# scroll-tech/scroll-prover

Hardware: AMD Instinct MI355X
Metric: BN254 MSM G1-adds/sec at k=26 (higher is better)
Workload: dtype u32 (9x29-bit limbs of 254-bit Montgomery integers; v_mad_u64_u32); 1 GPU; BN254 G1 Pippenger MSM, 2^26 uniform random scalars x synthetic SRS points, inputs resident in HBM; point-range shards over 1 GPU(s), RCCL all-gather of 96-B partials; log_n=26, window_bits=22, windows=12, parallelism=point-range x1, one rank per GPU, srs_window_tables=True

## Files before the change

include/mi355zk.h:

```cpp
#ifndef MI355ZK_H
#define MI355ZK_H
#include <stdint.h>
#ifdef __cplusplus
extern "C" {
#endif

#define MI355_OK 0
#define MI355_EBADARG 1
#define MI355_ENODEVICE 2
#define MI355_EOOM 3
#define MI355_EHIP 4
#define MI355_ERCCL 5

int mi355_init(int device_id);
int mi355_init_multi(const int *device_ids, int n_devices);
int mi355_device_count(int *n_out);
int mi355_shutdown(void);
const char *mi355_last_error(void);
const char *mi355_version(void);
int mi355_set_stream(void *hip_stream);
int mi355_reset_stream(void);
int mi355_synchronize(void);

int mi355_buf_alloc(uint64_t bytes, int device_slot, void **dev_ptr_out);
// ... 63 lines not shown
int mi355_fr_vec_mul_periodic_dev(void *data_dev, uint64_t n, const void *table_host, uint32_t period);
int mi355_fr_gate_eval_dev(void *dst_dev, const void *const *polys_dev, uint32_t n_polys, const void *coeffs_fr_host, const uint32_t *term_len,
                           uint32_t n_terms, const uint32_t *factor_poly, const int32_t *factor_rot, uint64_t n, int accumulate);
int mi355_fr_interleave_dev(void *dst_dev, const void *const *parts_dev, uint32_t q_parts, uint64_t n);
int mi355_fr_batch_invert_dev(void *data_dev, uint64_t n);
int mi355_fr_kate_division_dev(void *dst_dev, const void *poly_dev, uint64_t n, const void *z);
int mi355_fr_prefix_product_dev(void *dst_dev, const void *src_dev, uint64_t n, void *total_out_host);
int mi355_fr_prefix_sum_dev(void *dst_dev, const void *src_dev, uint64_t n, void *total_out_host);
int mi355_fr_lookup_multiplicities_dev(void *m_dev, uint64_t n, const void *table_dev, uint64_t table_rows, const void *const *inputs_dev,
                                       uint32_t n_inputs, uint64_t input_rows, uint32_t flags, uint64_t *missing_out);

int mi355_eval_polynomial_dev(const void *poly_dev, uint64_t n, const void *point, void *out_fr_host);
int mi355_eval_polynomial_batch_dev(const void *const *polys_dev, uint32_t batch, uint64_t n, const void *points, void *out_fr_host);
int mi355_eval_polynomial_host(const void *poly_host, uint64_t n, const void *point, void *out_fr_host);

int mi355_srs_setup_dev(void *g_dev, void *g_lagrange_dev, uint32_t k, const void *tau, const void *omega);
int mi355_g1_fixed_base_mul_dev(void *points_affine_dev, const void *scalars_dev, uint64_t n);

int mi355_g2_mul_host(const void *p_g2affine_host, const void *scalar_fr, void *out_g2affine_host);
int mi355_msm_g2_adhoc_host(const void *bases_g2affine_host, const void *scalars_host, uint64_t n, void *out_g2affine_host);
int mi355_msm_g2_dev(const void *bases_g2affine_dev, const void *scalars_dev, uint64_t n, void *out_g2affine_host);
int mi355_msm_g2_batch_dev(const void *bases_g2affine_dev, const void *const *scalars_dev, uint32_t batch, uint64_t n, void *out_g2affine_host);

int mi355_g1_fft_dev(void *points_jac_dev, uint32_t log_n, const void *omega);
int mi355_g1_fft_host(void *points_jac_host, uint32_t log_n, const void *omega);
int mi355_g_to_lagrange_dev(const void *g_affine_dev, void *g_lagrange_affine_dev, uint32_t log_n, const void *omega_inv, const void *n_inv);
int mi355_srs_downsize(uint64_t g_handle, uint32_t k, const void *omega_inv, const void *n_inv, uint64_t *g_lagrange_handle_out);
int mi355_srs_read_host(uint64_t handle, uint64_t offset, uint64_t n, void *out_affine_host);

int mi355_profile_enable(int on);
int mi355_profile_get(const char *name, double *ms_out, uint64_t *launches_out);
int mi355_profile_reset(void);
int mi355_msm_last_plan(int *c_out, int *windows_out, uint64_t *entries_out);
int mi355_msm_last_run(int *devices_out, const char **exchange_out, int *shared_tables_out, int *host_slices_out);

int mi355_debug_ws_read(const char *role, uint64_t offset, void *dst_host, uint64_t bytes);

#ifdef __cplusplus
}
#endif
#endif
```

scroll-prover_amd/_capi.py:

```python
from __future__ import annotations

import ctypes as C
import os

HERE = os.path.dirname(os.path.abspath(__file__))
LIB_PATH = os.environ.get("MI355ZK_LIB") or os.path.join(HERE, "libmi355zk.so")

OK, EBADARG, ENODEVICE, EOOM, EHIP, ERCCL = 0, 1, 2, 3, 4, 5
_vp, _u64, _u32, _int = C.c_void_p, C.c_uint64, C.c_uint32, C.c_int

SIGNATURES = {
    "mi355_init": (_int, [_int]),
    "mi355_init_multi": (_int, [C.POINTER(_int), _int]),
    "mi355_device_count": (_int, [C.POINTER(_int)]),
    "mi355_shutdown": (_int, []),
    "mi355_last_error": (C.c_char_p, []),
    "mi355_version": (C.c_char_p, []),
    "mi355_set_stream": (_int, [_vp]),
    "mi355_reset_stream": (_int, []),
    "mi355_synchronize": (_int, []),
    "mi355_buf_alloc": (_int, [_u64, _int, C.POINTER(_vp)]),
    "mi355_buf_free": (_int, [_vp]),
    "mi355_buf_trim": (_int, []),
    "mi355_buf_slot": (_int, [_vp, C.POINTER(_int)]),
# ... 45 lines not shown
    "mi355_ntt_fr_batch_host": (_int, [C.POINTER(_vp), _u32, _u32, _vp, _vp]),
    "mi355_ntt_fr_batch_dev": (_int, [C.POINTER(_vp), _u32, _u32, _vp, _vp]),
    "mi355_coset_ntt_fr_batch_dev": (_int, [C.POINTER(_vp), C.POINTER(_vp), _u32, _u32, _vp, _vp]),
    "mi355_fr_gate_eval_dev": (_int, [_vp, C.POINTER(_vp), _u32, _vp, C.POINTER(_u32), _u32, C.POINTER(_u32), C.POINTER(C.c_int32), _u64, _int]),
    "mi355_fr_interleave_dev": (_int, [_vp, C.POINTER(_vp), _u32, _u64]),
    "mi355_fr_vec_axpy_dev": (_int, [_vp, _vp, _vp, _vp, _u64]),
    "mi355_fr_vec_op_dev": (_int, [_int, _vp, _vp, _vp, _u64]),
    "mi355_fr_vec_mul_periodic_dev": (_int, [_vp, _u64, _vp, _u32]),
    "mi355_g1_fft_dev": (_int, [_vp, _u32, _vp]),
    "mi355_g1_fft_host": (_int, [_vp, _u32, _vp]),
    "mi355_g_to_lagrange_dev": (_int, [_vp, _vp, _u32, _vp, _vp]),
    "mi355_srs_load_params_file": (_int, [C.c_char_p, _u32, C.POINTER(_u32), C.POINTER(_u64), C.POINTER(_u64), _vp, _vp]),
    "mi355_srs_downsize": (_int, [_u64, _u32, _vp, _vp, C.POINTER(_u64)]),
    "mi355_srs_read_host": (_int, [_u64, _u64, _u64, _vp]),
    "mi355_fr_kate_division_dev": (_int, [_vp, _vp, _u64, _vp]),
    "mi355_fr_batch_invert_dev": (_int, [_vp, _u64]),
    "mi355_fr_prefix_product_dev": (_int, [_vp, _vp, _u64, _vp]),
    "mi355_fr_prefix_sum_dev": (_int, [_vp, _vp, _u64, _vp]),
    "mi355_fr_lookup_multiplicities_dev": (_int, [_vp, _u64, _vp, _u64, C.POINTER(_vp), _u32, _u64, _u32, C.POINTER(_u64)]),
    "mi355_eval_polynomial_dev": (_int, [_vp, _u64, _vp, _vp]),
    "mi355_eval_polynomial_batch_dev": (_int, [C.POINTER(_vp), _u32, _u64, _vp, _vp]),
    "mi355_eval_polynomial_host": (_int, [_vp, _u64, _vp, _vp]),
    "mi355_srs_setup_dev": (_int, [_vp, _vp, _u32, _vp, _vp]),
    "mi355_g1_fixed_base_mul_dev": (_int, [_vp, _vp, _u64]),
    "mi355_g2_mul_host": (_int, [_vp, _vp, _vp]),
    "mi355_msm_g2_adhoc_host": (_int, [_vp, _vp, _u64, _vp]),
    "mi355_msm_g2_dev": (_int, [_vp, _vp, _u64, _vp]),
    "mi355_msm_g2_batch_dev": (_int, [_vp, C.POINTER(_vp), _u32, _u64, _vp]),
    "mi355_profile_enable": (_int, [_int]),
    "mi355_profile_get": (_int, [C.c_char_p, C.POINTER(C.c_double), C.POINTER(_u64)]),
    "mi355_profile_reset": (_int, []),
    "mi355_debug_ws_read": (_int, [C.c_char_p, _u64, _vp, _u64]),
    "mi355_msm_last_plan": (_int, [C.POINTER(_int), C.POINTER(_int), C.POINTER(_u64)]),
    "mi355_msm_last_run": (_int, [C.POINTER(_int), C.POINTER(C.c_char_p), C.POINTER(_int), C.POINTER(_int)]),
}


class Mi355Error(RuntimeError):
    def __init__(self, code: int, msg: str):
        super().__init__(f"mi355zk error {code}: {msg}")
        self.code = code


_lib = None


def lib() -> C.CDLL:
    global _lib
    if _lib is None:
        if not os.path.exists(LIB_PATH):
            raise Mi355Error(ENODEVICE, f"{LIB_PATH} is missing: run __graft_entry__.build() (hipcc --offload-arch=gfx950); there is no CPU fallback")
        try:
            import torch
        except Exception:
            pass
        _lib = C.CDLL(LIB_PATH)
        for name, (res, args) in SIGNATURES.items():
            fn = getattr(_lib, name)
            fn.restype, fn.argtypes = res, args
    return _lib


def check(rc: int) -> None:
    if rc != OK:
        raise Mi355Error(rc, lib().mi355_last_error().decode())

# ... 38 lines not shown
```

scroll-prover_amd/csrc/lib_common.hpp:

```cpp
#pragma once
#include <hip/hip_runtime.h>
#include <stdio.h>
#include <stdlib.h>
#include <string.h>
#include <algorithm>
#include <atomic>
#include <chrono>
#include <map>
#include <memory>
#include <mutex>
#include <string>
#include <thread>
#include <condition_variable>
#include <unordered_map>
#include <vector>

#include "../../include/mi355zk.h"
#include "fp.hpp"
#include "g1.hpp"
#include "g1_29.hpp"
#include "ntt_types.hpp"

namespace mi355 {
using namespace zk;
// ... 34 lines not shown

struct Span { std::string name; hipEvent_t a, b; };
struct Ctx {
  bool inited = false;
  int slot = 0;
  std::vector<Span> spans;
  void *comm = nullptr;
  hipEvent_t ev_xchg = nullptr;
  hipEvent_t ev_xchg2 = nullptr;
  hipStream_t copy_stream = nullptr; hipEvent_t ev_copy[4] = {nullptr, nullptr, nullptr, nullptr};
  hipEvent_t ev_up_fork = nullptr;
  hipEvent_t ev_up[8] = {nullptr, nullptr, nullptr, nullptr, nullptr, nullptr, nullptr, nullptr}; uint32_t up_next = 0;
  uint32_t host_slice_min_log = 22;
  uint32_t host_batch_overlap = 1;
  uint32_t host_chunks = 8;
  int device = -1;
  hipDeviceProp_t prop;
  hipStream_t own_stream = nullptr, stream = nullptr;
  hipStream_t aux_stream[2] = {nullptr, nullptr};
  hipEvent_t ev_fork = nullptr;
  MsmSlot msm_slot[2];
  std::vector<const fe_t *> polys_stage;
  uint32_t msm_chunks = 1;
  uint32_t msm_chunk_min_log = 23;
  int last_chunks = 1;
  std::map<std::string, Buf> ws;
  std::map<std::string, NttPlan> ntt_plans;
  g1_affine_t *fixed_base_table = nullptr;
  uint32_t sort_t2 = 0;
  uint32_t seg_factor = 16;
  uint32_t sort_fb = 11;
  uint32_t sort_split = 1;
  uint32_t reduce_chains = 131072;
  uint32_t seg_fill = 40, seg_fill_segfix = 40;
  uint32_t seg_min = 16;
  uint32_t fixup_mode = 2;
  uint32_t fixup_huge_min = 2048;
  uint32_t fixup_serial_max = 32;
  uint32_t fixup_lanes_max_log = 17;
  uint32_t tail_coop_mask = 15;
  uint32_t tail_coop_max = 65536;
  uint32_t reduce_min_chunk = 4;
  uint32_t sort_t1 = 16384;
  uint32_t ntt_direct2_max_log = 25;
  uint32_t ntt_coset_fold_max_log = 26;
  uint32_t ntt_direct2_min_log = 0;
  uint32_t ntt_fold_scale = 1;
  uint32_t ntt_batch_max_log = 22;
  uint32_t ntt_two_level_max_log = 18;
  uint32_t ntt_tile_log = 11;
  bool profiling = false;
  bool trace = false;
  std::map<std::string, Prof> prof;
  int last_c = 0, last_w = 0; uint64_t last_entries = 0; bool last_shared = false; int last_host_slices = 1;
};

constexpr int MAX_DEV = 16;
extern std::mutex g_ctx_mu[MAX_DEV];
extern std::mutex g_upload_mu[MAX_DEV];
extern Ctx g_ctx[MAX_DEV];
extern int g_ndev;
extern bool g_dup_devices;
extern uint32_t g_shard_min_log;
extern bool g_peer_ok[MAX_DEV][MAX_DEV];
extern bool g_force_exchange;
extern thread_local Ctx *g_cur;
#define g (*::mi355::g_cur)
// ... 118 lines not shown
```

scroll-prover_amd/csrc/lib_msm.hip:

```cpp
#define ZK_FRSCAN_DEVICE_ONLY 1
#include "msm.hpp"
#define ZK_G2_DEVICE_ONLY 1
#include "msm_g2.hpp"
#include "lib_common.hpp"

namespace mi355 {

static_assert(sizeof(fe_t) == 32 && sizeof(g1_affine_t) == 64 && sizeof(g1_jac_t) == 96, "ABI element sizes");
static_assert(sizeof(g1_xyzz_t) == 128 && sizeof(g1_xyzz29_t) == 144, "device record sizes (workspace layout, 16-byte vector accesses)");

int msm_tu_init_device() {
  HIPCHK(hipFuncSetAttribute((const void *)k_sort_l1_scatter_split<24>, hipFuncAttributeMaxDynamicSharedMemorySize, 160 * 1024));
  HIPCHK(hipFuncSetAttribute((const void *)k_sort_l1_scatter_split<16>, hipFuncAttributeMaxDynamicSharedMemorySize, 160 * 1024));
  HIPCHK(hipFuncSetAttribute((const void *)k_sort_l1_scatter_split<8>, hipFuncAttributeMaxDynamicSharedMemorySize, 160 * 1024));
  HIPCHK(hipFuncSetAttribute((const void *)k_sort_l2_scatter_split<16>, hipFuncAttributeMaxDynamicSharedMemorySize, 160 * 1024));
  HIPCHK(hipFuncSetAttribute((const void *)k_sort_l2_scatter_split<8>, hipFuncAttributeMaxDynamicSharedMemorySize, 160 * 1024));
  return MI355_OK;
}

double msm_cost(uint64_t n, int c, bool shared) { const double W = (MSM_SCALAR_BITS + c - 1) / c, nb = (double)(1ull << (c - 1)); return 1.18 * W * (double)n + 8.2 * nb * (shared ? 1.0 : W) + (shared ? 0.0 : 3.0e7); }

int choose_c(uint64_t n) {
  if (t_opts.force_c) return t_opts.force_c;
  double best = 1e300; int best_c = 8;
  for (int c = 4; c <= g_auto_max_c; c++) {
    const double W = (MSM_SCALAR_BITS + c - 1) / c, nb = (double)(1ull << (c - 1));
    if (W * nb * sizeof(g1_xyzz29_t) > 6.0e9) continue;
    const double cost = msm_cost(n, c, false);
    if (cost < best) { best = cost; best_c = c; }
  }
  return best_c;
}

struct PreTable { const g1_affine_t *table = nullptr; uint64_t row_stride = 0; int c = 0, w = 0; };
const PreTable *pre_advance(const PreTable *pre, uint64_t lo, PreTable &store) {
  if (!pre) return nullptr;
  store = *pre; if (store.table) store.table += lo;
  return &store;
}

struct MsmShape { bool shared; uint32_t c, W, fb, cb_bits, regions; uint64_t emax, nbuckets; };
int msm_shape(uint64_t n, uint32_t M, const PreTable *pre, MsmShape &o, const MsmShape *forced = nullptr) {
  if (forced) { o.c = forced->c; o.shared = forced->shared; }
  else {
    o.c = (uint32_t)choose_c(n);
    o.shared = pre && pre->table && !t_opts.force_c && !t_opts.no_tables && msm_cost(n, pre->c, true) <= msm_cost(n, (int)o.c, false) && ((uint64_t)pre->w << log2_ceil(n)) < (1ull << 31);
    if (o.shared) o.c = (uint32_t)pre->c;
  }
  o.W = (MSM_SCALAR_BITS + o.c - 1) / o.c;
  o.emax = (uint64_t)M * n * o.W;
  const uint32_t kb = o.c - 1; uint32_t fb = kb < g.sort_fb ? kb : g.sort_fb; if (kb - fb > 11) fb = kb - 11;
  o.fb = fb; o.cb_bits = kb - fb;
  const uint64_t sets = (uint64_t)M * (o.shared ? 1 : o.W);
  o.nbuckets = sets << kb;
  const uint64_t regions = sets << o.cb_bits; o.regions = (uint32_t)std::min<uint64_t>(regions, 0xffffffffu);
  if (o.emax >= (1ull << 32)) return fail(MI355_EBADARG, "msm: n * windows must be < 2^32");
  if (o.nbuckets >= (1ull << 31)) return fail(MI355_EBADARG, "msm: too many buckets (split the batch)");
  if (regions * 4 > 48 * 1024) return fail(MI355_EBADARG, "msm: batch too large for the coarse histogram (split the batch)");
  if (o.fb > 12 || (1u << o.cb_bits) > SORT_MAX_BINS) return fail(MI355_EBADARG, "msm: window bits out of range for the sorter");
  return MI355_OK;
}

template <class G> bool msm_batch_must_split(uint64_t n, uint32_t M, const PreTable *pre) {
  MsmShape sh;
  return msm_shape(n, M, pre, sh) != MI355_OK || sh.emax > (1ull << 29) || sh.nbuckets * sizeof(typename G::rec_t) > (8ull << 30);
}

struct Roles {
  const char *prefix; std::string sfx;
  template <class T> int get(const char *name, size_t bytes, T *&ptr) const { return ws_get((std::string(prefix) + name + sfx).c_str(), bytes, (void **)&ptr); }
};

int msm_stage_polys(const fe_t *const *polys_host, uint32_t M, const Roles &ws, hipStream_t s, PolyPtrs &inl, const fe_t **&polys_dev) {
  if (M <= 8) { for (uint32_t m = 0; m < M; m++) inl.p[m] = polys_host[m]; return MI355_OK; }
  CHK(ws.get("polys", (size_t)M * sizeof(void *), polys_dev));
  g.polys_stage.assign(polys_host, polys_host + M);
  HIPCHK(hipMemcpyAsync(polys_dev, g.polys_stage.data(), (size_t)M * sizeof(void *), hipMemcpyHostToDevice, s));
  HIPCHK(hipStreamSynchronize(s));
  return MI355_OK;
}

struct AccPlan { uint32_t seg, blocks, tn; };
AccPlan msm_acc_plan(uint64_t emax) {
  const uint64_t want_threads = (uint64_t)g.prop.multiProcessorCount * 256 * g.seg_factor;
  uint64_t seg = (emax + want_threads - 1) / want_threads; if (seg < 16) seg = 16; if (seg > 4096) seg = 4096;
  const uint32_t blocks = ceil_div(ceil_div(emax, seg), 256);
  return {(uint32_t)seg, blocks, blocks * 256};
}
uint32_t msm_seg_arg(uint32_t seg, uint32_t fill_pct) { return seg | (std::min(g.seg_min, seg) << 13) | ((fill_pct / 2) << 26); }
MsmPlan msm_plan(const MsmShape &sh, uint64_t n, uint32_t M, uint32_t seg) {
  MsmPlan P; P.n = (uint32_t)n; P.c = sh.c; P.windows = sh.W; P.nb = 1u << (sh.c - 1); P.seg = seg; P.batch = M;
  return P;
}

template <class G, class F> void with_lanes(bool quad, F &&launch) {
  if constexpr (G::QUAD) { if (quad) { launch(std::integral_constant<int, 4>{}); return; } }
  launch(std::integral_constant<int, 1>{});
}

template <class G> int msm_segfix_levels(const int32_t *part_id, const typename G::rec_t *part, uint32_t tn, typename G::rec_t *buckets, hipStream_t s, const Roles &ws) {
  using rec_t = typename G::rec_t;
  uint32_t N = 2 * tn; const uint32_t waves1 = ceil_div(N, 64);
  const size_t cap = (size_t)2 * waves1 + (size_t)waves1 / 8 + 512;
  int32_t *lv_ids; rec_t *lv_recs;
  CHK(ws.get("segfix_ids", cap * 4, lv_ids)); CHK(ws.get("segfix_recs", cap * sizeof(rec_t), lv_recs));
  const int32_t *cur_ids = part_id; const rec_t *cur_recs = part; size_t used = 0;
  while (N > 64) {
    const uint32_t waves = ceil_div(N, 64);
    hipLaunchKernelGGL(k_msm_segfix<G>, dim3(ceil_div(N, 256)), dim3(256), 0, s, cur_ids, cur_recs, N, buckets, lv_ids + used, lv_recs + used, 0);
    cur_ids = lv_ids + used; cur_recs = lv_recs + used; used += (size_t)2 * waves; N = 2 * waves;
  }
  hipLaunchKernelGGL(k_msm_segfix<G>, dim3(1), dim3(64), 0, s, cur_ids, cur_recs, N, buckets, (int32_t *)nullptr, (rec_t *)nullptr, 1);
  return MI355_OK;
}

template <class G> int msm_reduce_tail(const MsmShape &sh, uint32_t M, const typename G::rec_t *buckets, typename G::out_t *out_dev, bool normalise, hipStream_t s, const Roles &ws) {
  using rec_t = typename G::rec_t;
  const uint32_t nb = 1u << (sh.c - 1), wpp = sh.shared ? 1 : sh.W, sets = M * wpp;
  uint32_t chunk = 64; while (chunk > nb) chunk >>= 1;
  while (chunk > g.reduce_min_chunk && (uint64_t)(nb / chunk) * sets < g.reduce_chains) chunk >>= 1;
  const uint32_t chunks_per_set = nb / chunk, nchunks = chunks_per_set * sets;
  rec_t *chunk_out, *tree_a, *tree_b, *window_sums;
// ... 65 lines not shown
      Scope s1(g2 ? "g2_sort_l1" : "sort_l1", s);
      const uint32_t CBp = ((1u << S.cb_bits) + 1) & ~1u;
      const size_t lds1 = (size_t)(3 * CBp + 32 + SORT_SPLIT_TMAX) * 4 + (size_t)S.t1 * 6;
      if (S.t1 == 24576) hipLaunchKernelGGL(k_sort_l1_scatter_split<24>, dim3(tiles1 * vwindows), dim3(1024), lds1, s, enc, coarse_cursor, pairs_lo, pairs_hi, S);
      else if (S.t1 == 16384) hipLaunchKernelGGL(k_sort_l1_scatter_split<16>, dim3(tiles1 * vwindows), dim3(1024), lds1, s, enc, coarse_cursor, pairs_lo, pairs_hi, S);
      else hipLaunchKernelGGL(k_sort_l1_scatter_split<8>, dim3(tiles1 * vwindows), dim3(1024), lds1, s, enc, coarse_cursor, pairs_lo, pairs_hi, S);
    }
    hipLaunchKernelGGL(k_sort_tile_prefix, dim3(1), dim3(SCAN_BLOCK), 0, s, coarse_off, tile_start, S);
    { Scope s2(g2 ? "g2_sort_hist" : "sort_hist", s);
    hipLaunchKernelGGL(k_sort_l2_hist_split, dim3(l2_tiles_max), dim3(256), 0, s, (const uint16_t *)pairs_hi, coarse_off, tile_start, hist, S); }
    hipLaunchKernelGGL(k_scan_partial, dim3(scan_blocks), dim3(SCAN_BLOCK), 0, s, hist, scan_sums, scan_n);
    hipLaunchKernelGGL(k_scan_block_sums, dim3(1), dim3(SCAN_BLOCK), 0, s, scan_sums, scan_blocks);
    hipLaunchKernelGGL(k_scan_final, dim3(scan_blocks), dim3(SCAN_BLOCK), 0, s, hist, scan_sums, offsets, cursor, scan_n);
    {
      Scope s3(g2 ? "g2_sort_l2" : "sort_l2", s);
      const size_t lds2 = (size_t)(3 * (1u << S.fb) + 32) * 4 + (size_t)S.t2 * 6;
      if (S.t2 == 8192) hipLaunchKernelGGL(k_sort_l2_scatter_split<8>, dim3(l2_tiles_max), dim3(1024), lds2, s, (const uint32_t *)pairs_lo, (const uint16_t *)pairs_hi, coarse_off, tile_start, cursor, sorted, S);
      else hipLaunchKernelGGL(k_sort_l2_scatter_split<16>, dim3(l2_tiles_max), dim3(1024), lds2, s, (const uint32_t *)pairs_lo, (const uint16_t *)pairs_hi, coarse_off, tile_start, cursor, sorted, S);
    }
  }
  return MI355_OK;
}

struct MsmStreams { hipStream_t a, b, c; };

int msm_enqueue(const g1_affine_t *bases, const PolyPtrs &inl, const fe_t *const *polys_dev, uint32_t M, uint64_t n, g1_jac_t *out_dev, const PreTable *pre, MsmSlot &slot,
                const MsmStreams &st, bool normalise, const MsmShape *forced = nullptr, uint32_t set_index = 0, uint32_t set_count = 1, bool skip_tail = false) {
  const bool piped = st.a != st.b;
  const Roles ws{G1Ops::ROLE, slot.id ? "#" + std::to_string(slot.id) : std::string()};
  MsmShape sh; CHK(msm_shape(n, M, pre, sh, forced));
  const bool shared = sh.shared;
  if (shared) bases = pre->table;
  const uint64_t emax = sh.emax;
  const AccPlan ap = msm_acc_plan(emax);
  const MsmPlan P = msm_plan(sh, n, M, ap.seg);
  const bool segfix = g.fixup_mode == 1 || (g.fixup_mode == 2 && (uint32_t)sh.nbuckets >= (1u << 19) && (uint64_t)P.seg * sh.nbuckets >= emax);
  const uint32_t seg_arg = msm_seg_arg(P.seg, segfix ? g.seg_fill_segfix : g.seg_fill);
  const uint32_t nbuckets = (uint32_t)sh.nbuckets;
  const uint32_t acc_blocks = ap.blocks, tn = ap.tn;
  uint32_t *offsets, *sorted;
  g1_xyzz29_t *buckets, *part; int32_t *part_id;
  CHK(ws.get("offsets", ((size_t)nbuckets + 1) * 4, offsets));
  CHK(ws.get("sorted", emax * 4, sorted));
  CHK(ws.get("buckets", (size_t)nbuckets * set_count * sizeof(g1_xyzz29_t), buckets));
  buckets += (size_t)nbuckets * set_index;
  CHK(ws.get("part", (size_t)tn * 2 * sizeof(g1_xyzz29_t), part));
  CHK(ws.get("part_id", (size_t)tn * 2 * 4, part_id));
  const uint32_t big_cap = tn / g.fixup_serial_max + 2;
  uint32_t *big_list; CHK(ws.get("big_list", ((size_t)big_cap * 3 + 1) * 4, big_list));
  uint32_t *big_count = big_list + (size_t)big_cap * 3;
  const uint32_t huge_cap = tn / FIXUP_HUGE_MIN + 2;
  uint32_t *huge_list, *huge_count; g1_xyzz29_t *huge_part;
  CHK(ws.get("huge_list", ((size_t)huge_cap * 3 + 1) * 4, huge_list)); huge_count = huge_list + (size_t)huge_cap * 3;
  CHK(ws.get("huge_part", (size_t)huge_cap * FIXUP_SLICES * sizeof(g1_xyzz29_t), huge_part));

  {
    hipStream_t s = st.a;
    if (piped && slot.used) { HIPCHK(hipStreamWaitEvent(s, slot.acc_done, 0)); HIPCHK(hipStreamWaitEvent(s, slot.red_done, 0)); }
    CHK(msm_sort_stage(inl, polys_dev, M, n, sh, P, offsets, sorted, s));
    if (piped) { HIPCHK(hipEventRecord(slot.sorted, s)); HIPCHK(hipStreamWaitEvent(st.b, slot.sorted, 0)); }
  }
  {
    hipStream_t s = st.b;
    if (piped && slot.used) HIPCHK(hipStreamWaitEvent(s, slot.red_done, 0));
    {
      Scope sc("msm_accumulate", s);
      HIPCHK(hipMemsetAsync(buckets, 0, (size_t)nbuckets * sizeof(g1_xyzz29_t), s));
      hipLaunchKernelGGL(k_msm_accumulate, dim3(acc_blocks), dim3(256), 0, s, bases, sorted, offsets, nbuckets, buckets, part, part_id, seg_arg, log2_ceil(n), shared ? pre->row_stride : (uint64_t)0);
    }
    if (piped) { HIPCHK(hipEventRecord(slot.acc_done, s)); HIPCHK(hipStreamWaitEvent(st.c, slot.acc_done, 0)); }
  }
  {
    hipStream_t s = st.c;
    Scope sc("msm_reduce", s);
    HIPCHK(hipMemsetAsync(big_count, 0, 4, s));
    HIPCHK(hipMemsetAsync(huge_count, 0, 4, s));
    if (segfix) CHK(msm_segfix_levels<G1Ops>(part_id, part, tn, buckets, s, ws));
    else {
      auto fixup = [&](auto kernel, uint64_t threads) {
        hipLaunchKernelGGL(kernel, dim3(ceil_div(threads, 256)), dim3(256), 0, s, offsets, nbuckets, buckets, part, part_id, seg_arg, tn, big_list, big_count, big_cap, huge_list, huge_count, huge_cap, g.fixup_serial_max, g.fixup_huge_min);
      };
      if ((uint64_t)nbuckets * 4 <= g.tail_coop_max && (g.tail_coop_mask & 1u)) fixup(k_msm_fixup<4, 4>, (uint64_t)nbuckets * 16);
      else if (nbuckets <= (1u << g.fixup_lanes_max_log)) fixup(k_msm_fixup<4, 1>, (uint64_t)nbuckets * 4);
      else fixup(k_msm_fixup<1, 1>, nbuckets);
      hipLaunchKernelGGL(k_msm_fixup_big, dim3(big_cap), dim3(256), 0, s, buckets, part, part_id, big_list, big_count);
      hipLaunchKernelGGL(k_msm_fixup_huge, dim3(huge_cap * FIXUP_SLICES), dim3(256), 0, s, part, part_id, huge_list, huge_count, huge_part, huge_cap);
      hipLaunchKernelGGL(k_msm_fixup_huge_fold, dim3(huge_cap), dim3(64), 0, s, buckets, huge_list, huge_count, (const g1_xyzz29_t *)huge_part);
    }
    if (!skip_tail) CHK(msm_reduce_tail<G1Ops>(sh, M, buckets, out_dev, normalise, s, ws));
  }
  if (piped) HIPCHK(hipEventRecord(slot.red_done, st.c));
  slot.used = true;
  HIPCHK(hipGetLastError());
  g.last_c = (int)P.c; g.last_w = (int)P.windows; g.last_entries += emax; g.last_shared = shared;
  return MI355_OK;
}

uint32_t msm_chunks_for(uint32_t M, uint64_t n) {
  if (g.msm_chunks <= 1 || M != 1 || n < (1ull << g.msm_chunk_min_log)) return 1;
  uint32_t k = g.msm_chunks;
  while (k > 1 && n / k < ((1ull << g.msm_chunk_min_log) >> 2)) k--;
  return k;
}

int msm_deliver(CallTrace &tr, const g1_jac_t *out_dev, uint32_t M, void *out_host, void *out_dev_user, hipStream_t s, const char *what, uint32_t count) {
  if (out_dev_user) {
    HIPCHK(hipMemcpyAsync(out_dev_user, out_dev, (size_t)M * sizeof(g1_jac_t), hipMemcpyDeviceToDevice, s));
    if (g.profiling) resolve_spans();
    tr.done(" (device result)");
    return MI355_OK;
  }
  HIPCHK(hipMemcpyAsync(out_host, out_dev, (size_t)M * sizeof(g1_jac_t), hipMemcpyDeviceToHost, s));
  HIPCHK(hipStreamSynchronize(s));
  resolve_spans();
  { char buf[64]; snprintf(buf, sizeof buf, " %s=%u c=%d W=%d", what, count, g.last_c, g.last_w); tr.done(buf); }
  return MI355_OK;
}

int msm_batch_impl(const g1_affine_t *bases, const fe_t *const *polys_host, uint32_t M, uint64_t n, void *out_host, const PreTable *pre, void *out_dev_user = nullptr, bool accumulate_plan = false) {
  if (M == 0) return MI355_OK;
  if (n == 0) {
    if (out_dev_user) { HIPCHK(hipMemsetAsync(out_dev_user, 0, (size_t)M * sizeof(g1_jac_t), g.stream)); return MI355_OK; }
    memset(out_host, 0, (size_t)M * sizeof(g1_jac_t)); return MI355_OK;
  }
  if (n >= (1ull << 31)) return fail(MI355_EBADARG, "msm: n must be < 2^31");
  if (M > 1 && msm_batch_must_split<G1Ops>(n, M, pre)) {
    const uint32_t h = M / 2;
    CHK(msm_batch_impl(bases, polys_host, h, n, out_host, pre, out_dev_user, accumulate_plan));
    return msm_batch_impl(bases, polys_host + h, M - h, n, out_host ? (char *)out_host + (size_t)h * sizeof(g1_jac_t) : nullptr, pre,
                          out_dev_user ? (char *)out_dev_user + (size_t)h * sizeof(g1_jac_t) : nullptr, true);
  }
  const uint32_t K = msm_chunks_for(M, n);
  if (!accumulate_plan) { g.last_entries = 0; g.last_host_slices = 1; }
  CallTrace tr("msm_g1", (uint64_t)M * n, 96.0);
  g1_jac_t *out_dev; const fe_t **polys_dev = nullptr;
  CHK(ws_get("msm.out", (size_t)(K + 1) * M * sizeof(g1_jac_t), (void **)&out_dev));
  hipStream_t s = g.stream;
  Scope total("msm_total", s);
  PolyPtrs inl{};
  if (K == 1) {
    CHK(msm_stage_polys(polys_host, M, Roles{G1Ops::ROLE, ""}, s, inl, polys_dev));
    MsmStreams st{s, s, s};
    CHK(msm_enqueue(bases, inl, polys_dev, M, n, out_dev, pre, g.msm_slot[0], st, t_opts.normalise));
  } else {
    std::vector<uint64_t> lo(K + 1);
    for (uint32_t k = 0; k <= K; k++) lo[k] = n * k / K;
    HIPCHK(hipEventRecord(g.ev_fork, s));
    HIPCHK(hipStreamWaitEvent(g.aux_stream[0], g.ev_fork, 0)); HIPCHK(hipStreamWaitEvent(g.aux_stream[1], g.ev_fork, 0));
// ... 50 lines not shown
    HIPCHK(hipEventRecord(g.ev_copy[k & 3], g.copy_stream));
    HIPCHK(hipStreamWaitEvent(s, g.ev_copy[k & 3], 0));
    PreTable pk; const PreTable *pp = pre_advance(pre, lo, pk);
    inl.p[0] = sc + lo;
    CHK(msm_enqueue(bases + lo, inl, nullptr, 1, hi - lo, out_dev, pp, g.msm_slot[0], st, t_opts.normalise, &shape, k, K, true));
  }
  g.msm_slot[0].used = false;
  g1_xyzz29_t *buckets; CHK(ws_get("msm.buckets", (size_t)shape.nbuckets * K * sizeof(g1_xyzz29_t), (void **)&buckets));
  {
    Scope sc2("msm_reduce", s);
    hipLaunchKernelGGL(k_msm_bucket_fold, dim3(ceil_div(shape.nbuckets, 256)), dim3(256), 0, s, buckets, (uint32_t)shape.nbuckets, K);
    CHK(msm_reduce_tail<G1Ops>(shape, 1, buckets, out_dev, t_opts.normalise, s, Roles{G1Ops::ROLE, ""}));
  }
  total.close();
  g.last_chunks = (int)K; g.last_host_slices = (int)K;
  return msm_deliver(tr, out_dev, 1, out_host, out_dev_user, s, "host slices", K);
}

static int msm_g2_impl(const g2_affine_t *bases, const fe_t *const *polys, uint32_t M, uint64_t n, void *out_host, bool accumulate_plan = false) {
  if (M == 0) return MI355_OK;
  if (n == 0) { memset(out_host, 0, (size_t)M * sizeof(g2_affine_t)); return MI355_OK; }
  if (n >= (1ull << 31)) return fail(MI355_EBADARG, "msm_g2: n must be < 2^31");
  if (M > 1 && msm_batch_must_split<G2Ops>(n, M, nullptr)) {
    const uint32_t h = M / 2;
    CHK(msm_g2_impl(bases, polys, h, n, out_host, accumulate_plan));
    return msm_g2_impl(bases, polys + h, M - h, n, (char *)out_host + (size_t)h * sizeof(g2_affine_t), true);
  }
  MsmShape sh; CHK(msm_shape(n, M, nullptr, sh));
  if (!accumulate_plan) { g.last_entries = 0; g.last_host_slices = 1; }
  CallTrace tr("msm_g2", (uint64_t)M * n, 160.0);
  hipStream_t s = g.stream;
  Scope total("msm_g2_total", s);
  const Roles ws{G2Ops::ROLE, ""};
  const AccPlan ap = msm_acc_plan(sh.emax);
  const MsmPlan P = msm_plan(sh, n, M, ap.seg);
  const uint32_t nbuckets = (uint32_t)sh.nbuckets;
  PolyPtrs inl{}; const fe_t **polys_dev = nullptr;
  CHK(msm_stage_polys(polys, M, ws, s, inl, polys_dev));
  uint32_t *offsets, *sorted; g2_xyzz_t *buckets, *part; int32_t *part_id;
  CHK(ws.get("offsets", ((size_t)nbuckets + 1) * 4, offsets));
  CHK(ws.get("sorted", sh.emax * 4, sorted));
  CHK(ws.get("buckets", (size_t)nbuckets * sizeof(g2_xyzz_t), buckets));
  CHK(ws.get("part", (size_t)ap.tn * 2 * sizeof(g2_xyzz_t), part));
  CHK(ws.get("part_id", (size_t)ap.tn * 2 * 4, part_id));
  CHK(msm_sort_stage(inl, polys_dev, M, n, sh, P, offsets, sorted, s, true));
  {
    Scope sc("msm_g2_accumulate", s);
    HIPCHK(hipMemsetAsync(buckets, 0, (size_t)nbuckets * sizeof(g2_xyzz_t), s));
    hipLaunchKernelGGL(k_msm_g2_accumulate, dim3(ap.blocks), dim3(256), 0, s, bases, sorted, offsets, nbuckets, buckets, part, part_id, msm_seg_arg(P.seg, 100));
  }
  {
    Scope sc("msm_g2_fixup", s);
    CHK(msm_segfix_levels<G2Ops>(part_id, part, ap.tn, buckets, s, ws));
  }
  g2_affine_t *out_dev; CHK(ws.get("out", (size_t)M * sizeof(g2_affine_t), out_dev));
  {
    Scope sc("msm_g2_reduce", s);
    CHK(msm_reduce_tail<G2Ops>(sh, M, buckets, out_dev, true, s, ws));
  }
  total.close();
  HIPCHK(hipMemcpyAsync(out_host, out_dev, (size_t)M * sizeof(g2_affine_t), hipMemcpyDeviceToHost, s));
  HIPCHK(hipStreamSynchronize(s));
  resolve_spans();
  g.last_c = (int)P.c; g.last_w = (int)P.windows; g.last_entries += sh.emax; g.last_shared = false; g.last_chunks = 1;
  { char buf[64]; snprintf(buf, sizeof buf, " batch=%u c=%d W=%d", M, g.last_c, g.last_w); tr.done(buf); }
  return MI355_OK;
}
// ... 408 lines not shown
  const fe_t *poly = sc;
  return msm_batch_impl(bs, &poly, 1, n, out_g1_host, nullptr);
  });
}
int mi355_g1_sum_host(const void *pts_host, uint64_t n, void *out_g1_host) {
  return guarded([&]() -> int {
  DevGuard lk(0);
  CHK(need_init());
  if (!out_g1_host || (n && !pts_host) || n > (1u << 20)) return fail(MI355_EBADARG, "g1_sum: bad argument");
  g1_jac_t *dev; CHK(ws_get("io.g1sum", (n + 1) * sizeof(g1_jac_t), (void **)&dev));
  if (n) HIPCHK(hipMemcpyAsync(dev + 1, pts_host, n * sizeof(g1_jac_t), hipMemcpyHostToDevice, g.stream));
  hipLaunchKernelGGL(k_g1_sum, dim3(1), dim3(64), 0, g.stream, dev + 1, (uint32_t)n, dev);
  HIPCHK(hipGetLastError());
  HIPCHK(hipMemcpyAsync(out_g1_host, dev, sizeof(g1_jac_t), hipMemcpyDeviceToHost, g.stream));
  HIPCHK(hipStreamSynchronize(g.stream));
  return MI355_OK;
  });
}
int mi355_msm_set_window_bits(int c) {
  return guarded([&]() -> int {
  if (c == -1) { t_opts.force_c = 0; t_opts.no_tables = true; return MI355_OK; }
  if (c != 0 && (c < 2 || c > MSM_MAX_C)) return fail(MI355_EBADARG, "window bits must be 0 (auto), -1 (auto, no window tables) or in [2, 24]");
  t_opts.force_c = c; t_opts.no_tables = false; return MI355_OK;
  });
}
int mi355_msm_set_normalise(int on) { t_opts.normalise = on != 0; return MI355_OK; }
int mi355_msm_last_plan(int *c_out, int *windows_out, uint64_t *entries_out) {
  return guarded([&]() -> int {
  DevGuard lk(0);
  const Ctx &p = g_ctx[0];
  if (c_out) *c_out = p.last_c; if (windows_out) *windows_out = p.last_w; if (entries_out) *entries_out = p.last_entries; return MI355_OK;
  });
}
int mi355_msm_last_run(int *devices_out, const char **exchange_out, int *shared_tables_out, int *host_slices_out) {
  return guarded([&]() -> int {
  DevGuard lk(0);
  if (devices_out) *devices_out = g_last_devices; if (exchange_out) *exchange_out = g_last_exchange;
  if (shared_tables_out) *shared_tables_out = g_ctx[0].last_shared ? 1 : 0; if (host_slices_out) *host_slices_out = g_ctx[0].last_host_slices;
  return MI355_OK;
  });
}

int mi355_msm_g2_adhoc_host(const void *bases_g2affine_host, const void *scalars_host, uint64_t n, void *out_g2affine_host) {
  return guarded([&]() -> int {
  MsmGuard lk;
  CHK(need_init());
  if (!out_g2affine_host || (n && (!scalars_host || !bases_g2affine_host))) return fail(MI355_EBADARG, "msm_g2: null pointer");
  if (n >= (1ull << 31)) return fail(MI355_EBADARG, "msm_g2: n must be < 2^31");
  fe_t *sc = nullptr; g2_affine_t *bs = nullptr;
  if (n) {
    CHK(ws_get("io.scalars", n * sizeof(fe_t), (void **)&sc)); CHK(ws_get("io.g2_bases", n * sizeof(g2_affine_t), (void **)&bs));
    HIPCHK(hipMemcpyAsync(sc, scalars_host, n * sizeof(fe_t), hipMemcpyHostToDevice, g.stream));
    HIPCHK(hipMemcpyAsync(bs, bases_g2affine_host, n * sizeof(g2_affine_t), hipMemcpyHostToDevice, g.stream));
  }
  const fe_t *p = sc;
  return msm_g2_run(bs, &p, 1, n, out_g2affine_host);
  });
}
static int g2_dev_operand(const void *p) {
  if (slot_of(p, true) != 0) return fail(MI355_EBADARG, "msm_g2: bases and scalars must live on the primary device (G2 MSMs run on one device)");
  return MI355_OK;
}
int mi355_msm_g2_dev(const void *bases_g2affine_dev, const void *scalars_dev, uint64_t n, void *out_g2affine_host) {
  return guarded([&]() -> int {
  MsmGuard lk;
  CHK(need_init());
// ... 62 lines not shown
```

scroll-prover_amd/csrc/msm.hpp:

```cpp
#pragma once
#include "fp_asm.hpp"
#include "g1_29.hpp"
#include "frscan.hpp"

namespace zk {

#if defined(__HIPCC__)

struct MsmPlan {
  uint32_t n;
  uint32_t c;
  uint32_t windows;
  uint32_t nb;
  uint32_t seg;
  uint32_t batch;
};

__device__ __forceinline__ g1_affine_t load_affine(const g1_affine_t *p) {
  g1_affine_t r; r.x = g_load(&p->x); r.y = g_load(&p->y); return r;
}
__device__ __forceinline__ g1_affine_t load_affine_nt(const g1_affine_t *p) {
  const uint32_t *q = reinterpret_cast<const uint32_t *>(p); g1_affine_t r;
#pragma unroll
  for (int i = 0; i < 8; i++) { r.x.l[i] = __builtin_nontemporal_load(q + i); r.y.l[i] = __builtin_nontemporal_load(q + 8 + i); }
// ... 370 lines not shown
      if (b_start >= start) G::store(&bucket_sums[b], acc);
      else { G::store(&part[2 * (uint64_t)t], acc); id_first = (int32_t)b; }
      acc = G::identity();
      b++; b_start = b_end; b_end = offsets[b + 1];
      if (pos >= b_end) {
        uint32_t l2 = b, h2 = nbuckets;
        while (h2 - l2 > 1) { const uint32_t mid = (l2 + h2) >> 1; if (offsets[mid] <= pos) l2 = mid; else h2 = mid; }
        b = l2; b_start = offsets[b]; b_end = offsets[b + 1];
      }
    }
    bases.madd(acc, p, (ent >> 31) != 0);
    ent = ent_next; p = p_next;
  }
  if (b_start >= start && b_end <= end) G::store(&bucket_sums[b], acc);
  else if (b_start < start) { G::store(&part[2 * (uint64_t)t], acc); id_first = (int32_t)b; }
  else { G::store(&part[2 * (uint64_t)t + 1], acc); id_last = (int32_t)b; }
  part_id[2 * t] = id_first; part_id[2 * t + 1] = id_last;
}
struct G1Bases {
  using base_t = g1_affine_t;
  const g1_affine_t *__restrict__ bases; uint32_t nshift; uint64_t row_stride;
  __device__ __forceinline__ const g1_affine_t *base_of(uint32_t e) const {
    const uint32_t gi = e & 0x7fffffffu;
    if (row_stride == 0) return &bases[gi];
    const uint32_t w = gi >> nshift;
    return &bases[(uint64_t)w * row_stride + (gi & ((1u << nshift) - 1))];
  }
  __device__ __forceinline__ g1_affine_t load(uint32_t e) const { return load_affine(base_of(e)); }
  __device__ __forceinline__ void madd(g1_xyzz29_t &acc, const g1_affine_t &p, bool neg) const { g1_xyzz29_madd(acc, p, neg); }
};
struct G1AccOps : G1Ops {
  static __device__ __forceinline__ void store(rec_t *p, rec_t v) { g1_xyzz29_negx_to_plain(v); store_xyzz29(p, v); }
};
__global__ void __launch_bounds__(256) k_msm_accumulate(const g1_affine_t *__restrict__ bases, const uint32_t *__restrict__ sorted, const uint32_t *__restrict__ offsets,
                                                        uint32_t nbuckets, g1_xyzz29_t *__restrict__ bucket_sums, g1_xyzz29_t *__restrict__ part, int32_t *__restrict__ part_id, uint32_t seg_arg,
                                                        uint32_t nshift, uint64_t row_stride) {
  msm_segment_walk<G1AccOps>(G1Bases{bases, nshift, row_stride}, sorted, offsets, nbuckets, bucket_sums, part, part_id, seg_arg, blockIdx.x * blockDim.x + threadIdx.x, gridDim.x * blockDim.x);
}

constexpr uint32_t FIXUP_SERIAL_MAX = 32, FIXUP_HUGE_MIN = 2048, FIXUP_SLICES = 64;
template <int Q = 1> __device__ __forceinline__ void fixup_take29(g1_xyzz29_t &acc, const g1_xyzz29_t *__restrict__ part, const int32_t *__restrict__ part_id, uint32_t t, uint32_t b) {
  if (part_id[2 * t] == (int32_t)b) g1_vadd<Q>(acc, load_xyzz29(&part[2 * (uint64_t)t]));
  else if (part_id[2 * t + 1] == (int32_t)b) g1_vadd<Q>(acc, load_xyzz29(&part[2 * (uint64_t)t + 1]));
}
template <uint32_t FIXUP_LANES, int Q = 1> __global__ void __launch_bounds__(256) k_msm_fixup(const uint32_t *__restrict__ offsets, uint32_t nbuckets, g1_xyzz29_t *__restrict__ bucket_sums,
                                                   const g1_xyzz29_t *__restrict__ part, const int32_t *__restrict__ part_id, uint32_t seg_arg, uint32_t acc_threads,
                                                   uint32_t *__restrict__ big_list, uint32_t *__restrict__ big_count, uint32_t big_cap,
                                                   uint32_t *__restrict__ huge_list, uint32_t *__restrict__ huge_count, uint32_t huge_cap, uint32_t serial_max, uint32_t huge_min) {
  const uint32_t gid = (blockIdx.x * blockDim.x + threadIdx.x) / Q, b = gid / FIXUP_LANES, sub = gid % FIXUP_LANES;
  const bool lead = (threadIdx.x & (Q - 1)) == 0;
  const uint32_t seg = msm_seg_eff(offsets[nbuckets], acc_threads, seg_arg);
  g1_xyzz29_t acc = g1_xyzz29_identity();
  bool mine = false;
  if (b < nbuckets) {
    const uint32_t s = offsets[b], e = offsets[b + 1];
    if (e != s) {
      const uint32_t t0 = s / seg, t1 = (e - 1) / seg;
      if (t0 != t1) {
        if (t1 - t0 > serial_max) {
          if (sub == 0 && lead) {
            if (huge_cap && t1 - t0 >= huge_min) {
              const uint32_t idx = atomicAdd(huge_count, 1u);
              if (idx < huge_cap) { huge_list[3 * idx] = b; huge_list[3 * idx + 1] = t0; huge_list[3 * idx + 2] = t1; }
            } else {
              const uint32_t idx = atomicAdd(big_count, 1u);
              if (idx < big_cap) { big_list[3 * idx] = b; big_list[3 * idx + 1] = t0; big_list[3 * idx + 2] = t1; }
            }
// ... 239 lines not shown
```

Before: 12.52 billion G1-adds/s.

## Size MSM accumulate grid to whole rounds of resident workgroups

Pins k_msm_accumulate to a fixed waves-per-EU occupancy and queries how many workgroups fit per CU at init. The accumulate plan then picks a segment length so the grid is an integer number of full resident waves, which avoids a partial tail round. The segment fill percentage is derived from the round count instead of a fixed 40. This adds a new query API for the launch shape. Forcing waves_per_eu=4 may push the compiler to spill registers in the 29-bit-limb point-add code.

```diff
diff --git a/include/mi355zk.h b/include/mi355zk.h
--- a/include/mi355zk.h
+++ b/include/mi355zk.h
@@ -119,6 +119,7 @@
 int mi355_profile_get(const char *name, double *ms_out, uint64_t *launches_out);
 int mi355_profile_reset(void);
 int mi355_msm_last_plan(int *c_out, int *windows_out, uint64_t *entries_out);
+int mi355_msm_last_launch(uint32_t *seg_out, uint32_t *workgroups_out, uint32_t *resident_out);
 int mi355_msm_last_run(int *devices_out, const char **exchange_out, int *shared_tables_out, int *host_slices_out);
 
 int mi355_debug_ws_read(const char *role, uint64_t offset, void *dst_host, uint64_t bytes);
diff --git a/scroll-prover_amd/_capi.py b/scroll-prover_amd/_capi.py
--- a/scroll-prover_amd/_capi.py
+++ b/scroll-prover_amd/_capi.py
@@ -101,6 +101,7 @@
     "mi355_profile_reset": (_int, []),
     "mi355_debug_ws_read": (_int, [C.c_char_p, _u64, _vp, _u64]),
     "mi355_msm_last_plan": (_int, [C.POINTER(_int), C.POINTER(_int), C.POINTER(_u64)]),
+    "mi355_msm_last_launch": (_int, [C.POINTER(_u32), C.POINTER(_u32), C.POINTER(_u32)]),
     "mi355_msm_last_run": (_int, [C.POINTER(_int), C.POINTER(C.c_char_p), C.POINTER(_int), C.POINTER(_int)]),
 }
 
diff --git a/scroll-prover_amd/csrc/lib_common.hpp b/scroll-prover_amd/csrc/lib_common.hpp
--- a/scroll-prover_amd/csrc/lib_common.hpp
+++ b/scroll-prover_amd/csrc/lib_common.hpp
@@ -90,7 +90,9 @@
   uint32_t sort_fb = 11;
   uint32_t sort_split = 1;
   uint32_t reduce_chains = 131072;
-  uint32_t seg_fill = 40, seg_fill_segfix = 40;
+  uint32_t seg_fill = 0, seg_fill_segfix = 0;
+  uint32_t acc_resident = 0;
+  uint32_t last_acc_seg = 0, last_acc_blocks = 0;
   uint32_t seg_min = 16;
   uint32_t fixup_mode = 2;
   uint32_t fixup_huge_min = 2048;
diff --git a/scroll-prover_amd/csrc/lib_msm.hip b/scroll-prover_amd/csrc/lib_msm.hip
--- a/scroll-prover_amd/csrc/lib_msm.hip
+++ b/scroll-prover_amd/csrc/lib_msm.hip
@@ -15,6 +15,10 @@
   HIPCHK(hipFuncSetAttribute((const void *)k_sort_l1_scatter_split<8>, hipFuncAttributeMaxDynamicSharedMemorySize, 160 * 1024));
   HIPCHK(hipFuncSetAttribute((const void *)k_sort_l2_scatter_split<16>, hipFuncAttributeMaxDynamicSharedMemorySize, 160 * 1024));
   HIPCHK(hipFuncSetAttribute((const void *)k_sort_l2_scatter_split<8>, hipFuncAttributeMaxDynamicSharedMemorySize, 160 * 1024));
+  int per_cu = 0;
+  HIPCHK(hipOccupancyMaxActiveBlocksPerMultiprocessor(&per_cu, (const void *)k_msm_accumulate, 256, 0));
+  if (per_cu < 1) return fail(MI355_EHIP, "msm: k_msm_accumulate has no resident workgroup on this device");
+  g.acc_resident = (uint32_t)g.prop.multiProcessorCount * std::min<uint32_t>((uint32_t)per_cu, (uint32_t)MSM_ACC_WAVES);
   return MI355_OK;
 }
 
@@ -80,14 +84,25 @@
   return MI355_OK;
 }
 
-struct AccPlan { uint32_t seg, blocks, tn; };
-AccPlan msm_acc_plan(uint64_t emax) {
+struct AccPlan { uint32_t seg, blocks, tn, rounds; };
+AccPlan msm_acc_plan(uint64_t emax, uint32_t resident) {
   const uint64_t want_threads = (uint64_t)g.prop.multiProcessorCount * 256 * g.seg_factor;
   uint64_t seg = (emax + want_threads - 1) / want_threads; if (seg < 16) seg = 16; if (seg > 4096) seg = 4096;
   const uint32_t blocks = ceil_div(ceil_div(emax, seg), 256);
-  return {(uint32_t)seg, blocks, blocks * 256};
+  if (resident && blocks >= 2 * (uint64_t)resident) {
+    uint32_t rounds = (uint32_t)((blocks + resident / 2) / resident);
+    if (rounds > 2 && (emax + (uint64_t)rounds * resident * 256 - 1) / ((uint64_t)rounds * resident * 256) < 16) rounds--;
+    const uint64_t tn = (uint64_t)rounds * resident * 256, seg_r = (emax + tn - 1) / tn;
+    if (seg_r >= 16 && seg_r <= 4096 && tn < (1ull << 31)) return {(uint32_t)seg_r, rounds * resident, (uint32_t)tn, rounds};
+  }
+  return {(uint32_t)seg, blocks, blocks * 256, 0};
 }
 uint32_t msm_seg_arg(uint32_t seg, uint32_t fill_pct) { return seg | (std::min(g.seg_min, seg) << 13) | ((fill_pct / 2) << 26); }
+uint32_t msm_fill_pct(uint32_t knob, const AccPlan &ap) {
+  if (knob) return knob;
+  if (ap.rounds < 2) return 40;
+  return std::min(100u, ((200u + ap.rounds - 1) / ap.rounds + 1) & ~1u);
+}
 MsmPlan msm_plan(const MsmShape &sh, uint64_t n, uint32_t M, uint32_t seg) {
   MsmPlan P; P.n = (uint32_t)n; P.c = sh.c; P.windows = sh.W; P.nb = 1u << (sh.c - 1); P.seg = seg; P.batch = M;
   return P;
@@ -219,10 +234,10 @@
   const bool shared = sh.shared;
   if (shared) bases = pre->table;
   const uint64_t emax = sh.emax;
-  const AccPlan ap = msm_acc_plan(emax);
+  const AccPlan ap = msm_acc_plan(emax, g.acc_resident);
   const MsmPlan P = msm_plan(sh, n, M, ap.seg);
   const bool segfix = g.fixup_mode == 1 || (g.fixup_mode == 2 && (uint32_t)sh.nbuckets >= (1u << 19) && (uint64_t)P.seg * sh.nbuckets >= emax);
-  const uint32_t seg_arg = msm_seg_arg(P.seg, segfix ? g.seg_fill_segfix : g.seg_fill);
+  const uint32_t seg_arg = msm_seg_arg(P.seg, msm_fill_pct(segfix ? g.seg_fill_segfix : g.seg_fill, ap));
   const uint32_t nbuckets = (uint32_t)sh.nbuckets;
   const uint32_t acc_blocks = ap.blocks, tn = ap.tn;
   uint32_t *offsets, *sorted;
@@ -280,6 +295,7 @@
   slot.used = true;
   HIPCHK(hipGetLastError());
   g.last_c = (int)P.c; g.last_w = (int)P.windows; g.last_entries += emax; g.last_shared = shared;
+  g.last_acc_seg = ap.seg; g.last_acc_blocks = ap.blocks;
   return MI355_OK;
 }
 
@@ -300,7 +316,7 @@
   HIPCHK(hipMemcpyAsync(out_host, out_dev, (size_t)M * sizeof(g1_jac_t), hipMemcpyDeviceToHost, s));
   HIPCHK(hipStreamSynchronize(s));
   resolve_spans();
-  { char buf[64]; snprintf(buf, sizeof buf, " %s=%u c=%d W=%d", what, count, g.last_c, g.last_w); tr.done(buf); }
+  { char buf[128]; snprintf(buf, sizeof buf, " %s=%u c=%d W=%d acc=%ux%u/%u", what, count, g.last_c, g.last_w, g.last_acc_blocks, g.last_acc_seg, g.acc_resident); tr.done(buf); }
   return MI355_OK;
 }
 
@@ -417,7 +433,7 @@
   hipStream_t s = g.stream;
   Scope total("msm_g2_total", s);
   const Roles ws{G2Ops::ROLE, ""};
-  const AccPlan ap = msm_acc_plan(sh.emax);
+  const AccPlan ap = msm_acc_plan(sh.emax, 0);
   const MsmPlan P = msm_plan(sh, n, M, ap.seg);
   const uint32_t nbuckets = (uint32_t)sh.nbuckets;
   PolyPtrs inl{}; const fe_t **polys_dev = nullptr;
@@ -892,6 +908,13 @@
   if (c_out) *c_out = p.last_c; if (windows_out) *windows_out = p.last_w; if (entries_out) *entries_out = p.last_entries; return MI355_OK;
   });
 }
+int mi355_msm_last_launch(uint32_t *seg_out, uint32_t *workgroups_out, uint32_t *resident_out) {
+  return guarded([&]() -> int {
+  DevGuard lk(0);
+  const Ctx &p = g_ctx[0];
+  if (seg_out) *seg_out = p.last_acc_seg; if (workgroups_out) *workgroups_out = p.last_acc_blocks; if (resident_out) *resident_out = p.acc_resident; return MI355_OK;
+  });
+}
 int mi355_msm_last_run(int *devices_out, const char **exchange_out, int *shared_tables_out, int *host_slices_out) {
   return guarded([&]() -> int {
   DevGuard lk(0);
diff --git a/scroll-prover_amd/csrc/msm.hpp b/scroll-prover_amd/csrc/msm.hpp
--- a/scroll-prover_amd/csrc/msm.hpp
+++ b/scroll-prover_amd/csrc/msm.hpp
@@ -426,7 +426,8 @@
 struct G1AccOps : G1Ops {
   static __device__ __forceinline__ void store(rec_t *p, rec_t v) { g1_xyzz29_negx_to_plain(v); store_xyzz29(p, v); }
 };
-__global__ void __launch_bounds__(256) k_msm_accumulate(const g1_affine_t *__restrict__ bases, const uint32_t *__restrict__ sorted, const uint32_t *__restrict__ offsets,
+constexpr int MSM_ACC_WAVES = 4;
+__global__ void __launch_bounds__(256) __attribute__((amdgpu_waves_per_eu(MSM_ACC_WAVES, MSM_ACC_WAVES))) k_msm_accumulate(const g1_affine_t *__restrict__ bases, const uint32_t *__restrict__ sorted, const uint32_t *__restrict__ offsets,
                                                         uint32_t nbuckets, g1_xyzz29_t *__restrict__ bucket_sums, g1_xyzz29_t *__restrict__ part, int32_t *__restrict__ part_id, uint32_t seg_arg,
                                                         uint32_t nshift, uint64_t row_stride) {
   msm_segment_walk<G1AccOps>(G1Bases{bases, nshift, row_stride}, sorted, offsets, nbuckets, bucket_sums, part, part_id, seg_arg, blockIdx.x * blockDim.x + threadIdx.x, gridDim.x * blockDim.x);
```

New measurement: 12.51 billion G1-adds/s (median of 2 runs). No clear change (-0.0%).
